# wooginawunan/multi-modal-uncertainty

Measured on AMD Instinct MI355X. Metric: image+text samples/sec/node, MMBT Food-101 bs=256 seq=512; ECE/NLL parity, higher is better.
Workload: dtype bf16

## Files before the change

multi-modal-uncertainty_amd/csrc/attention.hip:

```cpp
#include "mmu_common.h"
#include "mmu_internal.h"
#include <cstdlib>
#include <type_traits>
#include <utility>

namespace mmu {

constexpr float LOG2E = 1.4426950408889634f;
constexpr float LN2 = 0.6931471805599453f;
constexpr float NEG_INF = -__builtin_huge_valf();

static __device__ __forceinline__ uint32_t lowbias32(uint32_t x) {
  x ^= x >> 16; x *= 0x7feb352du; x ^= x >> 15; x *= 0x846ca68bu; x ^= x >> 16;
  return x;
}
static __device__ __forceinline__ uint32_t seed_for(uint64_t seed, int bh) {
  return lowbias32((uint32_t)seed ^ lowbias32((uint32_t)(seed >> 32) + 0x9E3779B9u * (uint32_t)(bh + 1)));
}
static __device__ __forceinline__ uint32_t drop_pair(uint32_t sbh, uint32_t q, uint32_t key, uint32_t Lp) {
  return lowbias32(((q * Lp + key) >> 1) ^ sbh);
}

static __device__ __forceinline__ float max3f(float a, float b, float c) {
  return __builtin_fmaxf(__builtin_fmaxf(a, b), c);
}
static __device__ __forceinline__ uint32_t bfi(uint32_t m, uint32_t a, uint32_t b) {
  return (m & a) | (~m & b);
}
static __device__ __forceinline__ uint32_t keepmask(uint32_t w, uint32_t pos) {
  uint32_t r;
  asm("v_bfe_i32 %0, %1, %2, 1" : "=v"(r) : "v"(w), "v"(pos));
  return r;
}
template <typename F, int... R>
static __device__ __forceinline__ void static_for(F&& f, std::integer_sequence<int, R...>) {
  (f(std::integral_constant<int, R>{}), ...);
}
template <int POS>
static __device__ __forceinline__ uint32_t keepmask(uint32_t w) {
  uint32_t r;
  asm("v_bfe_i32 %0, %1, %2, 1" : "=v"(r) : "v"(w), "n"(POS));
  return r;
}
static __host__ __device__ __forceinline__ uint32_t drop_thr(float p) { return (uint32_t)(p * 65536.0f + 0.5f); }

static __device__ __forceinline__ int fsw(int r) { return (((r >> 1) & 1) << 2) | ((r >> 3) & 3); }
static __device__ __forceinline__ int tile_off(int row, int chunk) { return row * 128 + ((chunk ^ fsw(row)) << 4); }

static __device__ __forceinline__ bf16x8 row_frag(const char* s, int row0, int ks, int l) {
  return *(const bf16x8*)(s + tile_off(row0 + (l & 31), 2 * ks + (l >> 5)));
}
static __device__ __forceinline__ bf16x8 tr_frag(const char* s, int row0, int col0, int l) {
  const int g = l >> 4, i = l & 15, q = i >> 2, p = i & 3, h = g >> 1;
  const int col = col0 + 16 * (g & 1) + 4 * p;
  const int r0 = row0 + 4 * h + q, r1 = r0 + 8;
  const int cb = col * 2;
  const char* a0 = s + tile_off(r0, cb >> 4) + (cb & 15);
  const char* a1 = s + tile_off(r1, cb >> 4) + (cb & 15);
  bf16x4 lo = __builtin_amdgcn_ds_read_tr16_b64_v4bf16((MMU_LDS(bf16x4)*)a0);
  bf16x4 hi = __builtin_amdgcn_ds_read_tr16_b64_v4bf16((MMU_LDS(bf16x4)*)a1);
  return __builtin_shufflevector(lo, hi, 0, 1, 2, 3, 4, 5, 6, 7);
}
static __device__ __forceinline__ bf16x8 acc_frag(const f32x16& a, int s) {
  bf16x8 r;
#pragma unroll
  for (int j = 0; j < 8; ++j) r[j] = f2bf(a[8 * s + j]);
  return r;
}
static __device__ __forceinline__ bf16x8 scale_frag(uint4 u, float sc) {
  bf16x8 v = *(bf16x8*)&u;
#pragma unroll
  for (int j = 0; j < 8; ++j) v[j] = f2bf(bf2f(v[j]) * sc);
  return v;
}

static __device__ __forceinline__ __amdgpu_buffer_rsrc_t urs(const void* base, int bytes) {
  const uint64_t a = (uint64_t)base;
  const uint32_t lo = __builtin_amdgcn_readfirstlane((uint32_t)a);
  const uint32_t hi = __builtin_amdgcn_readfirstlane((uint32_t)(a >> 32));
  const int n = __builtin_amdgcn_readfirstlane(bytes);
  return __builtin_amdgcn_make_buffer_rsrc((void*)(((uint64_t)hi << 32) | lo), 0, n, 0x00020000);
}

static __device__ __forceinline__ void dma16(__amdgpu_buffer_rsrc_t r, char* lds, uint32_t off) {
  __builtin_amdgcn_raw_ptr_buffer_load_lds(r, (MMU_LDS(void)*)lds, 16, off, 0, 0, 0);
}
static __device__ __forceinline__ __amdgpu_buffer_rsrc_t urs_at(const void* base, int bytes, int off) {
  return urs((const char*)base + off, bytes > off ? bytes - off : 0);
}
static __device__ __forceinline__ void dma4(__amdgpu_buffer_rsrc_t r, char* lds, uint32_t off) {
  __builtin_amdgcn_raw_ptr_buffer_load_lds(r, (MMU_LDS(void)*)lds, 4, off, 0, 0, 0);
}
static __device__ __forceinline__ void raw_barrier() {
  __builtin_amdgcn_s_barrier();
  asm volatile("" ::: "memory");
}

static __device__ __forceinline__ void block_coords(int& bx, int& bh) {
  const int gx = gridDim.x;
  const int wid = xcd_remap(blockIdx.y * gx + blockIdx.x, gx * gridDim.y);
  bh = wid / gx;
  bx = wid - bh * gx;
}

constexpr int FWD_NS = 2;
constexpr int FWD_TILE = 64 * 128;
constexpr int FWD_STAGE = 2 * FWD_TILE + 256;
constexpr int FWD_MAX_NKV = 9;

constexpr float DEFER_LOG2 = 8.0f;
constexpr uint32_t kDropMul24[8] = {0x9E3779u, 0x85EBCBu, 0xC2B2AFu, 0xA7D4EBu,
                                    0x965667u, 0xD3A265u, 0xFD7047u, 0xB55A4Fu};

static __device__ __forceinline__ uint32_t pair_draw(uint32_t hb, int i) {
  const uint32_t src = i ? __builtin_amdgcn_alignbit(hb, hb, 4 * i) : hb;
  const uint32_t x = __umul24(src, kDropMul24[i]);
  return x ^ (x >> 16);
}

static __device__ __forceinline__ int kperm(int i) {
  return (((i >> 2) & 1) << 4) | (((i >> 3) & 3) << 2) | (i & 3);
}

static __device__ __forceinline__ void drop_pair_zero(uint32_t hsh, uint32_t thr, uint32_t thr_hi, float e0,
                                                      float e1, float& o0, float& o1) {
  asm("v_cmp_le_u32 vcc, %[th], %[h]\n\t"
      "v_cndmask_b32 %[o1], 0, %[e1], vcc\n\t"
      "v_cmp_le_u16 vcc, %[t], %[h]\n\t"
      "v_cndmask_b32 %[o0], 0, %[e0], vcc"
      : [o0] "=&v"(o0), [o1] "=&v"(o1)
      : [e0] "v"(e0), [e1] "v"(e1), [h] "v"(hsh), [t] "s"(thr), [th] "s"(thr_hi)
      : "vcc");
}

static __device__ __forceinline__ void drop_pair_apply(uint32_t hsh, uint32_t thr, uint32_t thr_hi, float e0,
                                                       float e1, float& o0, float& o1, uint32_t& w) {
  asm("v_cmp_le_u32 vcc, %[th], %[h]\n\t"
      "v_cndmask_b32 %[o1], 0, %[e1], vcc\n\t"
      "v_addc_co_u32 %[w], vcc, %[w], %[w], vcc\n\t"
      "v_cmp_le_u16 vcc, %[t], %[h]\n\t"
      "v_cndmask_b32 %[o0], 0, %[e0], vcc\n\t"
      "v_addc_co_u32 %[w], vcc, %[w], %[w], vcc"
      : [o0] "=&v"(o0), [o1] "=&v"(o1), [w] "+v"(w)
      : [e0] "v"(e0), [e1] "v"(e1), [h] "v"(hsh), [t] "s"(thr), [th] "s"(thr_hi)
      : "vcc");
}

template <bool DROP, int WPE, bool NOHOIST, bool STORE = true>
__global__ __launch_bounds__(256) __attribute__((amdgpu_waves_per_eu(WPE))) void attn_fwd_v2_kernel(AttnParams p) {
  __shared__ __attribute__((aligned(16))) char smem[FWD_NS * FWD_STAGE + 4 * 32 * FWD_MAX_NKV * 8];
  uint64_t* kbuf_all = (uint64_t*)(smem + FWD_NS * FWD_STAGE);
  const int t = threadIdx.x, l = t & 63, l_ = l, h = l >> 5;
  const int w = __builtin_amdgcn_readfirstlane(t >> 6);
  int bx, bh;
  block_coords(bx, bh);
  const int b = bh / p.heads, hd = bh - b * p.heads;
  const int L = p.L, HD = p.heads * 64;
  const int q0w = bx * 128 + 32 * w, q = q0w + (l & 31);
  const bool wave_live = q0w < L;
  const bf16* base = p.qkv + (int64_t)b * L * p.ld_qkv + hd * 64;
  const uint32_t thr = drop_thr(p.drop_p), thr_hi = thr << 16;
  const int nkv = (L + 63) / 64;
  uint64_t* kbuf = kbuf_all + w * 32 * nkv;
  const bool store_bits = STORE && DROP && p.dropmask != nullptr;
  const uint32_t ctr = seed_for(mmu_eff_seed(p.seed, p.seed_off), bh) + 4u * (uint32_t)q * (uint32_t)nkv + 2u * (uint32_t)h;

  const void* kv_base = p.qkv + (int64_t)b * L * p.ld_qkv;
  const int kv_bytes = (int)(L * p.ld_qkv * 2);
  const void* m_base = p.keymask + (int64_t)b * L;
  bf16x8 qf[4];
#pragma unroll
  for (int ks = 0; ks < 4; ++ks) {
    uint4 u = q < L ? *(const uint4*)(base + (int64_t)q * p.ld_qkv + 16 * ks + 8 * h) : make_uint4(0, 0, 0, 0);
    qf[ks] = scale_frag(u, 0.125f);
// ... 106 lines not shown
      }
#pragma unroll
      for (int u = 0; u < 2; ++u) {
        if (PARTIAL && u == 1 && 64 * j + 32 * s2 + 8 >= L) break;
        const bf16x8 pf = acc_frag(sc[s2], u);
#pragma unroll
        for (int dt = 0; dt < 2; ++dt)
          o[dt] = __builtin_amdgcn_mfma_f32_32x32x16_bf16(tr_frag(Vs, 32 * s2 + 16 * u, 32 * dt, l), pf, o[dt], 0, 0, 0);
      }
    }
    if (store_bits) {
      const uint64_t mine = ((uint64_t)(wb[1] & 0xFFFFu) << (32 + 16 * h)) | ((uint64_t)(wb[0] & 0xFFFFu) << (16 * h));
      const uint32_t lo = (uint32_t)mine | (uint32_t)__shfl_xor((int)(uint32_t)mine, 32, 64);
      const uint32_t hi = (uint32_t)(mine >> 32) | (uint32_t)__shfl_xor((int)(uint32_t)(mine >> 32), 32, 64);
      if (h == 0) kbuf[(l & 31) * nkv + j] = ((uint64_t)hi << 32) | lo;
    }
  };

  asm volatile("s_waitcnt vmcnt(0)" ::: "memory");
  for (int j = 0; j < FWD_NS - 1 && j < nkv; ++j) issue(j);
  const int nfull = L / 64;
  auto step = [&](int j) {
    const int ahead = nkv - 1 - j < FWD_NS - 2 ? nkv - 1 - j : FWD_NS - 2;
    wait_for(ahead);
    raw_barrier();
    if (j + FWD_NS - 1 < nkv) issue(j + FWD_NS - 1);
  };
  static_assert(FWD_NS == 2, "the forward loop is unrolled by its ring depth");
  for (int j = 0; j < nfull; j += 2) {
    step(j);
    if (wave_live) tile(j, std::integral_constant<bool, false>{}, smem);
    if (j + 1 < nfull) {
      step(j + 1);
      if (wave_live) tile(j + 1, std::integral_constant<bool, false>{}, smem + FWD_STAGE);
    }
  }
  if (nfull < nkv) {
    step(nfull);
    if (wave_live) tile(nfull, std::integral_constant<bool, true>{}, smem + (nfull % FWD_NS) * FWD_STAGE);
  }
  raw_barrier();
  if (!wave_live) return;
  if (store_bits) {
    uint64_t* dst = p.dropmask + ((int64_t)bh * L + q0w) * nkv;
    const int rows = L - q0w < 32 ? L - q0w : 32;
    for (int i = l; i < rows * nkv; i += 64) dst[i] = kbuf[i];
  }
  const float l_run = (lsum[0] + lsum[1]) + (lsum[2] + lsum[3]);
  const float lsum_row = l_run + __shfl_xor(l_run, 32, 64);
  const float inv = (DROP ? 1.0f / (1.0f - p.drop_p) : 1.0f) / lsum_row;
  char* os = smem + w * 4096;
  const int qr = l & 31;
#pragma unroll
  for (int dt = 0; dt < 2; ++dt)
#pragma unroll
    for (int g = 0; g < 4; ++g) {
      const bf16x4 v = {f2bf(o[dt][4 * g] * inv), f2bf(o[dt][4 * g + 1] * inv), f2bf(o[dt][4 * g + 2] * inv),
                        f2bf(o[dt][4 * g + 3] * inv)};
      *(bf16x4*)(os + qr * 128 + (((4 * dt + g) ^ (qr & 7)) << 4) + 8 * h) = v;
    }
  if (h == 0 && q < L) p.lse[(int64_t)bh * L + q] = m_run + logf(lsum_row);
  asm volatile("s_waitcnt lgkmcnt(0)" ::: "memory");
  bf16* ob = p.out + hd * 64;
#pragma unroll
  for (int i = 0; i < 4; ++i) {
    const int r = (l >> 3) + 8 * i, c = l & 7;
    if (q0w + r < L)
      *(uint4*)(ob + ((int64_t)b * L + q0w + r) * p.ld_out + 8 * c) = *(const uint4*)(os + r * 128 + ((c ^ (r & 7)) << 4));
  }
}

void attention_fwd_launch(const AttnParams& p, hipStream_t s) {
  dim3 grid((p.L + 127) / 128, p.batch * p.heads);
  if (drop_thr(p.drop_p) && !p.dropmask) {
    hipLaunchKernelGGL((attn_fwd_v2_kernel<true, 3, true, false>), grid, dim3(256), 0, s, p);
  } else if (drop_thr(p.drop_p)) {
    hipLaunchKernelGGL((attn_fwd_v2_kernel<true, 2, false>), grid, dim3(256), 0, s, p);
  } else {
    hipLaunchKernelGGL((attn_fwd_v2_kernel<false, 3, false>), grid, dim3(256), 0, s, p);
  }
}

constexpr int DK_NS = 4;
constexpr int DK_TILE = 32 * 128;
constexpr int DK_ROWS = 32 * 4 + 32 * 4 + 32 * 8;
constexpr int DK_STAGE = 2 * DK_TILE + DK_ROWS;


template <bool DROP>
__global__ __launch_bounds__(128) __attribute__((amdgpu_waves_per_eu(2))) void attn_dkdv_dma_kernel(AttnParams p) {
  __shared__ __attribute__((aligned(16))) char smem[DK_NS * DK_STAGE];
  const int t = threadIdx.x, l = t & 63, h = l >> 5;
  const int w = __builtin_amdgcn_readfirstlane(t >> 6);
  int bx, bh;
  block_coords(bx, bh);
  const int b = bh / p.heads, hd = bh - b * p.heads;
  const int L = p.L, HD = p.heads * 64;
  const int k0w = bx * 64 + 32 * w, key = k0w + (l & 31);
  const bool wave_live = k0w < L, kv = key < L;
  const bool drop = DROP;
  const float zs = drop ? 1.0f / (1.0f - p.drop_p) : 1.0f;
  const int lane31 = l & 31;
  const int nkv = (L + 63) / 64;
  const float mkey = kv ? p.keymask[(int64_t)b * L + key] * LOG2E : NEG_INF;
  const bf16* base = p.qkv + (int64_t)b * L * p.ld_qkv + hd * 64;

  const void* q_base = p.qkv + (int64_t)b * L * p.ld_qkv;
  const int q_bytes = (int)(L * p.ld_qkv * 2);
  const void* do_base = p.dout + (int64_t)b * L * p.ld_do;
  const int do_bytes = (int)(L * p.ld_do * 2);
  const void* l_base = p.lse + (int64_t)bh * L;
  const void* d_base = p.delta + (int64_t)bh * L;
  const void* k_base = drop ? (const void*)(p.dropmask + (int64_t)bh * L * nkv) : nullptr;

  bf16x8 kf[4], vf[4];
#pragma unroll
  for (int ks = 0; ks < 4; ++ks) {
    uint4 u = kv ? *(const uint4*)(base + (int64_t)key * p.ld_qkv + HD + 16 * ks + 8 * h) : make_uint4(0, 0, 0, 0);
    uint4 v = kv ? *(const uint4*)(base + (int64_t)key * p.ld_qkv + 2 * HD + 16 * ks + 8 * h) : make_uint4(0, 0, 0, 0);
    kf[ks] = scale_frag(u, -0.125f);
    vf[ks] = *(bf16x8*)&v;
  }
  f32x16 dk[2], dv[2];
#pragma unroll
  for (int i = 0; i < 16; ++i) { dk[0][i] = 0.f; dk[1][i] = 0.f; dv[0][i] = 0.f; dv[1][i] = 0.f; }

  const int nq = (L + 31) / 32;
  uint32_t pc_off[4];
  const int ldr = w == 0 ? p.ld_qkv : p.ld_do;
#pragma unroll
  for (int pc = 0; pc < 4; ++pc) {
    const int row = 8 * pc + (l >> 3), c = (l & 7) ^ fsw(row);
    pc_off[pc] = (uint32_t)((row * ldr + hd * 64 + 8 * c) * 2);
  }
  const uint32_t row_off = (uint32_t)(16 * l), kw_off = (uint32_t)((((l >> 1) * nkv + bx) * 8) + 4 * (l & 1));
  auto issue = [&](int i) {
    char* st = smem + (i % DK_NS) * DK_STAGE;
    const int q0 = i * 32;
    if (w == 0) {
      const __amdgpu_buffer_rsrc_t rt = urs_at(q_base, q_bytes, q0 * p.ld_qkv * 2);
#pragma unroll
      for (int pc = 0; pc < 4; ++pc) dma16(rt, st + pc * 1024, pc_off[pc]);
      if (l < 8) {
        dma16(urs_at(l_base, L * 4, q0 * 4), st + 2 * DK_TILE, row_off);
        dma16(urs_at(d_base, L * 4, q0 * 4), st + 2 * DK_TILE + 128, row_off);
      }
    } else {
      const __amdgpu_buffer_rsrc_t rt = urs_at(do_base, do_bytes, q0 * p.ld_do * 2);
#pragma unroll
      for (int pc = 0; pc < 4; ++pc) dma16(rt, st + DK_TILE + pc * 1024, pc_off[pc]);
      dma4(urs_at(k_base, drop ? L * nkv * 8 : 0, q0 * nkv * 8), st + 2 * DK_TILE + 256, kw_off);
    }
  };
  auto wait_for = [&](int ahead) {
    if (w == 0) {
      if (ahead >= 2) asm volatile("s_waitcnt vmcnt(12)" ::: "memory");
      else if (ahead == 1) asm volatile("s_waitcnt vmcnt(6)" ::: "memory");
      else asm volatile("s_waitcnt vmcnt(0)" ::: "memory");
    } else {
      if (ahead >= 2) asm volatile("s_waitcnt vmcnt(10)" ::: "memory");
      else if (ahead == 1) asm volatile("s_waitcnt vmcnt(5)" ::: "memory");
      else asm volatile("s_waitcnt vmcnt(0)" ::: "memory");
    }
  };
  asm volatile("s_waitcnt vmcnt(0)" ::: "memory");
  for (int i = 0; i < DK_NS - 1 && i < nq; ++i) issue(i);
  auto qtile = [&](int i, auto sg_tag) {
    constexpr int SG = decltype(sg_tag)::value;
    const int ahead = nq - 1 - i < DK_NS - 2 ? nq - 1 - i : DK_NS - 2;
    wait_for(ahead);
    raw_barrier();
    if (i + DK_NS - 1 < nq) issue(i + DK_NS - 1);
    const char* st = smem + SG * DK_STAGE;
    const char* Qs = st;
    const char* Ds = st + DK_TILE;
    const float* lse = (const float*)(st + 2 * DK_TILE);
    const float* dlt = lse + 32;
    const uint32_t* kbit = (const uint32_t*)(st + 2 * DK_TILE + 256) + w;
    if (wave_live) {
      f32x4 l4[4], nd4[4];
      uint32_t kwr[16];
#pragma unroll
      for (int j = 0; j < 4; ++j) {
        l4[j] = *(const f32x4*)(lse + 8 * j + 4 * h);
        nd4[j] = *(const f32x4*)(dlt + 8 * j + 4 * h);
        if (DROP)
#pragma unroll
          for (int i2 = 0; i2 < 4; ++i2) kwr[4 * j + i2] = kbit[2 * (8 * j + 4 * h + i2)];
      }
      f32x16 sc, dp;
#pragma unroll
      for (int r = 0; r < 16; ++r) {
        sc[r] = l4[r >> 2][r & 3];
        dp[r] = nd4[r >> 2][r & 3];
      }
#pragma unroll
      for (int ks = 0; ks < 4; ++ks) {
        sc = __builtin_amdgcn_mfma_f32_32x32x16_bf16(row_frag(Qs, 0, ks, l), kf[ks], sc, 0, 0, 0);
        dp = __builtin_amdgcn_mfma_f32_32x32x16_bf16(row_frag(Ds, 0, ks, l), vf[ks], dp, 0, 0, 0);
      }
      f32x16 pz;
#pragma unroll
      for (int r = 0; r < 16; ++r) {
        const float pr = __builtin_amdgcn_exp2f(fmaf(sc[r], -LOG2E, mkey));
        if (DROP) {
          const uint32_t m = keepmask(kwr[r], lane31);
          pz[r] = __uint_as_float(m & __float_as_uint(pr));
          sc[r] = pr * __uint_as_float(bfi(m, __float_as_uint(dp[r]), __float_as_uint(nd4[r >> 2][r & 3])));
        } else {
          pz[r] = pr;
          sc[r] = pr * dp[r];
        }
      }
#pragma unroll
      for (int s2 = 0; s2 < 2; ++s2) {
        if (s2 == 1 && 32 * i + 16 >= L) break;
        bf16x8 pf = acc_frag(pz, s2), sf = acc_frag(sc, s2);
#pragma unroll
        for (int dt = 0; dt < 2; ++dt) {
          dv[dt] = __builtin_amdgcn_mfma_f32_32x32x16_bf16(pf, tr_frag(Ds, 16 * s2, 32 * dt, l), dv[dt], 0, 0, 0);
          dk[dt] = __builtin_amdgcn_mfma_f32_32x32x16_bf16(sf, tr_frag(Qs, 16 * s2, 32 * dt, l), dk[dt], 0, 0, 0);
        }
      }
    }
  };
  for (int i0 = 0; i0 < nq; i0 += DK_NS) {
    qtile(i0, std::integral_constant<int, 0>{});
    if (i0 + 1 < nq) qtile(i0 + 1, std::integral_constant<int, 1>{});
    if (i0 + 2 < nq) qtile(i0 + 2, std::integral_constant<int, 2>{});
    if (i0 + 3 < nq) qtile(i0 + 3, std::integral_constant<int, 3>{});
  }
  static_assert(DK_NS == 4, "the dK/dV loop is unrolled by its ring depth");
  const float dks = 0.125f * zs;
  if (p.colsum) {
    float* red = (float*)smem;
    raw_barrier();
#pragma unroll
    for (int dt = 0; dt < 2; ++dt) {
      float sk = 0.f, sv = 0.f;
#pragma unroll
      for (int r = 0; r < 16; ++r) {
        const bool ok = k0w + (r & 3) + 8 * (r >> 2) + 4 * h < L;
        sk += ok ? dk[dt][r] : 0.f;
        sv += ok ? dv[dt][r] : 0.f;
      }
      sk += __shfl_xor(sk, 32, 64);
      sv += __shfl_xor(sv, 32, 64);
      if (h == 0) {
        red[w * 128 + 32 * dt + l] = sk * dks;
        red[w * 128 + 64 + 32 * dt + l] = sv * zs;
      }
    }
    raw_barrier();
    if (t < 128) {
      const int nqb = (L + 127) / 128, nkb = (L + 63) / 64, B = p.batch;
      const float v = red[t] + red[128 + t];
      const int64_t row = (int64_t)nqb * B + (t < 64 ? 0 : (int64_t)nkb * B) + (int64_t)bx * B + b;
      p.colsum[row * HD + hd * 64 + (t & 63)] = v;
    }
  }
  if (!wave_live) return;
  bf16* outb = p.out + (int64_t)b * L * p.ld_out + hd * 64;
#pragma unroll
  for (int dt = 0; dt < 2; ++dt)
#pragma unroll
    for (int r = 0; r < 16; ++r) {
      const int kk = k0w + (r & 3) + 8 * (r >> 2) + 4 * h;
      if (kk < L) {
        const int64_t off = (int64_t)kk * p.ld_out + 32 * dt + (l & 31);
        outb[off + HD] = f2bf(dk[dt][r] * dks);
        outb[off + 2 * HD] = f2bf(dv[dt][r] * zs);
      }
    }
}

constexpr int DQ_NS = 3;
constexpr int DQ_TILE = 64 * 128;
constexpr int DQ_STAGE = 2 * DQ_TILE + 256 + 4 * 256;

__global__ __launch_bounds__(256) __attribute__((amdgpu_waves_per_eu(3))) void attn_dq_dma_kernel(AttnParams p) {
  __shared__ __attribute__((aligned(16))) char smem[DQ_NS * DQ_STAGE];
  const int t = threadIdx.x, l = t & 63, h = l >> 5;
  const int w = __builtin_amdgcn_readfirstlane(t >> 6);
  int bx, bh;
  block_coords(bx, bh);
  const int b = bh / p.heads, hd = bh - b * p.heads;
  const int L = p.L, HD = p.heads * 64;
  const int q0w = bx * 128 + 32 * w, q = q0w + (l & 31);
  const bool wave_live = q0w < L, qv = q < L;
  const bool drop = drop_thr(p.drop_p) != 0;
  const float zs = drop ? 1.0f / (1.0f - p.drop_p) : 1.0f;
  const int nkv = (L + 63) / 64;
  const bf16* base = p.qkv + (int64_t)b * L * p.ld_qkv + hd * 64;

  const void* kv_base = p.qkv + (int64_t)b * L * p.ld_qkv;
  const int kv_bytes = (int)(L * p.ld_qkv * 2);
  const void* m_base = p.keymask + (int64_t)b * L;
  const void* k_base = drop ? (const void*)(p.dropmask + (int64_t)bh * L * nkv) : nullptr;
  const int k_bytes = drop ? (int)(L * nkv * 8) : 0;

  bf16x8 qf[4], df[4];
  const bf16* dob = p.dout + ((int64_t)b * L + q) * p.ld_do + hd * 64;
#pragma unroll
  for (int ks = 0; ks < 4; ++ks) {
    uint4 u = qv ? *(const uint4*)(base + (int64_t)q * p.ld_qkv + 16 * ks + 8 * h) : make_uint4(0, 0, 0, 0);
    qf[ks] = scale_frag(u, 0.125f);
    uint4 v = qv ? *(const uint4*)(dob + 16 * ks + 8 * h) : make_uint4(0, 0, 0, 0);
    df[ks] = *(bf16x8*)&v;
  }
  float dsum = 0.f;
  {
    const bf16* ob = p.o + ((int64_t)b * L + q) * p.ld_o + hd * 64;
#pragma unroll
    for (int ks = 0; ks < 4; ++ks) {
      uint4 u = qv ? *(const uint4*)(ob + 16 * ks + 8 * h) : make_uint4(0, 0, 0, 0);
      const bf16x8 ov = *(bf16x8*)&u;
#pragma unroll
      for (int e = 0; e < 8; ++e) dsum = fmaf(bf2f(ov[e]), bf2f(df[ks][e]), dsum);
    }
    dsum += __shfl_xor(dsum, 32, 64);
    if (qv && h == 0) p.delta[(int64_t)bh * L + q] = -dsum / zs;
  }
  const float nlse2 = qv ? -p.lse[(int64_t)bh * L + q] * LOG2E : -__builtin_huge_valf();
  const float ndz = -dsum / zs;
  const uint32_t ndz_bits = __float_as_uint(ndz);
  f32x16 dq[2];
#pragma unroll
  for (int i = 0; i < 16; ++i) { dq[0][i] = 0.f; dq[1][i] = 0.f; }

  uint32_t kv_off[4];
#pragma unroll
  for (int pc = 0; pc < 4; ++pc) {
    const int piece = 4 * (w & 1) + pc;
    const int row = 8 * piece + (l >> 3), c = (l & 7) ^ fsw(row);
    kv_off[pc] = (uint32_t)((row * p.ld_qkv + (w < 2 ? HD : 2 * HD) + hd * 64 + 8 * c) * 2);
  }
  const uint32_t m_off = (uint32_t)(16 * l), kw_off = (uint32_t)(((q0w + (l >> 1)) * nkv * 8) + 4 * (l & 1));
  auto issue = [&](int j) {
    char* st = smem + (j % DQ_NS) * DQ_STAGE;
    const int k0 = j * 64;
    char* dst = st + (w < 2 ? 0 : DQ_TILE);
    const __amdgpu_buffer_rsrc_t rt = urs_at(kv_base, kv_bytes, k0 * p.ld_qkv * 2);
#pragma unroll
    for (int pc = 0; pc < 4; ++pc) dma16(rt, dst + (4 * (w & 1) + pc) * 1024, kv_off[pc]);
    if (w == 0 && l < 16) dma16(urs_at(m_base, L * 4, k0 * 4), st + 2 * DQ_TILE, m_off);
    dma4(urs_at(k_base, k_bytes, j * 8), st + 2 * DQ_TILE + 256 + w * 256, kw_off);
  };
  auto wait_for = [&](int ahead) {
    if (w == 0) {
      if (ahead >= 1) asm volatile("s_waitcnt vmcnt(6)" ::: "memory");
      else asm volatile("s_waitcnt vmcnt(0)" ::: "memory");
    } else {
      if (ahead >= 1) asm volatile("s_waitcnt vmcnt(5)" ::: "memory");
      else asm volatile("s_waitcnt vmcnt(0)" ::: "memory");
    }
  };
  asm volatile("s_waitcnt vmcnt(0)" ::: "memory");
  for (int j = 0; j < DQ_NS - 1 && j < nkv; ++j) issue(j);
  auto tile_step = [&](int j, auto sg_tag) {
    constexpr int SG = decltype(sg_tag)::value;
    const int ahead = nkv - 1 - j < DQ_NS - 2 ? nkv - 1 - j : DQ_NS - 2;
    wait_for(ahead);
    raw_barrier();
    if (j + DQ_NS - 1 < nkv) issue(j + DQ_NS - 1);
    const char* st = smem + SG * DQ_STAGE;
    const char* Ks = st;
    const char* Vs = st + DQ_TILE;
    const float* mk = (const float*)(st + 2 * DQ_TILE);
    const uint32_t* kwords = (const uint32_t*)(st + 2 * DQ_TILE + 256 + w * 256);
    if (wave_live) {
      const uint64_t kw = drop ? ((uint64_t)kwords[2 * (l & 31) + 1] << 32 | kwords[2 * (l & 31)]) : ~0ull;
      const uint64_t kwh = kw >> (4 * h);
#pragma unroll
      for (int st2 = 0; st2 < 2; ++st2) {
        if (st2 == 1 && 64 * j + 32 >= L) break;
        const uint32_t kw32 = (uint32_t)(kwh >> (32 * st2));
        f32x16 sc, dp;
#pragma unroll
        for (int g = 0; g < 4; ++g) {
          const f32x4 mv = *(const f32x4*)(mk + 32 * st2 + 8 * g + 4 * h);
#pragma unroll
          for (int e = 0; e < 4; ++e) {
            sc[4 * g + e] = mv[e];
            dp[4 * g + e] = ndz;
          }
        }
#pragma unroll
        for (int ks = 0; ks < 4; ++ks) {
          sc = __builtin_amdgcn_mfma_f32_32x32x16_bf16(row_frag(Ks, 32 * st2, ks, l), qf[ks], sc, 0, 0, 0);
          dp = __builtin_amdgcn_mfma_f32_32x32x16_bf16(row_frag(Vs, 32 * st2, ks, l), df[ks], dp, 0, 0, 0);
        }
        auto one = [&](auto r_tag) {
          constexpr int r = decltype(r_tag)::value;
          const float pr = __builtin_amdgcn_exp2f(fmaf(sc[r], LOG2E, nlse2));
          const uint32_t m = keepmask<(r & 3) + 8 * (r >> 2)>(kw32);
          sc[r] = pr * __uint_as_float(bfi(m, __float_as_uint(dp[r]), ndz_bits));
        };
        static_for(one, std::make_integer_sequence<int, 16>{});
#pragma unroll
        for (int s2 = 0; s2 < 2; ++s2) {
          bf16x8 sf = acc_frag(sc, s2);
#pragma unroll
          for (int dt = 0; dt < 2; ++dt)
            dq[dt] = __builtin_amdgcn_mfma_f32_32x32x16_bf16(tr_frag(Ks, 32 * st2 + 16 * s2, 32 * dt, l), sf, dq[dt],
                                                             0, 0, 0);
        }
      }
    }
    };
  for (int j0 = 0; j0 < nkv; j0 += DQ_NS) {
    tile_step(j0, std::integral_constant<int, 0>{});
    if (j0 + 1 < nkv) tile_step(j0 + 1, std::integral_constant<int, 1>{});
    if (j0 + 2 < nkv) tile_step(j0 + 2, std::integral_constant<int, 2>{});
  }
  if (p.colsum) {
    constexpr int RS = 68;
    static_assert(4 * 32 * RS * 4 <= DQ_NS * DQ_STAGE, "dQ column-sum rows exceed the ring's LDS");
    float* rows = (float*)smem;
    raw_barrier();
    float* mine = rows + w * 32 * RS + (l & 31) * RS;
    const float sc = qv ? 0.125f * zs : 0.f;
#pragma unroll
    for (int dt = 0; dt < 2; ++dt)
#pragma unroll
      for (int g = 0; g < 4; ++g)
        *(float4*)(mine + 32 * dt + 8 * g + 4 * h) =
            make_float4(dq[dt][4 * g] * sc, dq[dt][4 * g + 1] * sc, dq[dt][4 * g + 2] * sc, dq[dt][4 * g + 3] * sc);
    raw_barrier();
    if (t < 64) {
      float v = 0.f;
      for (int r = 0; r < 128; ++r) v += rows[r * RS + t];
      p.colsum[((int64_t)bx * p.batch + b) * HD + hd * 64 + t] = v;
    }
  }
  if (!qv) return;
  bf16* ob = p.out + ((int64_t)b * L + q) * p.ld_out + hd * 64;
#pragma unroll
  for (int dt = 0; dt < 2; ++dt)
#pragma unroll
    for (int g = 0; g < 4; ++g) {
      const float s = 0.125f * zs;
      bf16x4 v = {f2bf(dq[dt][4 * g] * s), f2bf(dq[dt][4 * g + 1] * s), f2bf(dq[dt][4 * g + 2] * s),
                  f2bf(dq[dt][4 * g + 3] * s)};
      *(bf16x4*)(ob + 32 * dt + 8 * g + 4 * h) = v;
    }
}

void attention_bwd_launch(const AttnParams& p, hipStream_t s) {
  hipLaunchKernelGGL(attn_dq_dma_kernel, dim3((p.L + 127) / 128, p.batch * p.heads), dim3(256), 0, s, p);
  if (drop_thr(p.drop_p))
    hipLaunchKernelGGL(attn_dkdv_dma_kernel<true>, dim3((p.L + 63) / 64, p.batch * p.heads), dim3(128), 0, s, p);
  else
    hipLaunchKernelGGL(attn_dkdv_dma_kernel<false>, dim3((p.L + 63) / 64, p.batch * p.heads), dim3(128), 0, s, p);
}

}
```

multi-modal-uncertainty_amd/csrc/capi.hip:

```cpp
#include <stdarg.h>
#include <stdio.h>
#include <map>
#include <tuple>
#include <mutex>
#include <string>
#include <vector>
#include "mmu_internal.h"
#include <cstdlib>
#include <cmath>

using namespace mmu;

static thread_local std::string g_err;

namespace mmu {
const uint64_t* g_seed_off = nullptr;
}

int mmu_set_seed_offset(const uint64_t* dev_counter) {
  g_seed_off = dev_counter;
  return 0;
}

static int fail(const char* fmt, ...) {
// ... 262 lines not shown
    splitk_epilogue_launch(pe, c_dtype == MMU_F32, tail_ws, m_main, tail_rows, tail_split, s);
  }
  if (cs_part) colsum_reduce_launch(cs_part, cs_parts, N, p.colsum, 1, s);
  if (p.splitk > 1) splitk_reduce_launch(p, (int)batch, s);
  if (timed) {
    (void)hipEventRecord(ev.second, s);
    std::lock_guard<std::mutex> lk(g_t.mu);
    g_t.used.push_back(ev);
    g_t.flops.push_back(2.0 * (double)M * (double)N * (double)K * (double)batch);
  }
  return check_launch("mmu_gemm");
}

int mmu_transpose_bf16_batched(const int64_t* jobs, int n_jobs, int64_t max_rows, int64_t max_cols,
                               mmu_stream_t stream) {
  if (!jobs || n_jobs <= 0 || n_jobs > 65535 || max_rows <= 0 || max_cols <= 0)
    return fail("mmu_transpose_bf16_batched: bad args");
  transpose_bf16_batched_launch(jobs, n_jobs, max_rows, max_cols, (hipStream_t)stream);
  return check_launch("mmu_transpose_bf16_batched");
}

int mmu_colsum_reduce(const float* partial, int64_t parts, int64_t N, float* out, int accumulate,
                      mmu_stream_t stream) {
  if (!partial || !out || parts <= 0 || N <= 0) return fail("mmu_colsum_reduce: bad args");
  colsum_reduce_launch(partial, parts, N, out, accumulate, (hipStream_t)stream);
  return check_launch("mmu_colsum_reduce");
}

int mmu_colsum_reduce_multi(int n, const float* const* partial, const int64_t* parts, float* const* out, int64_t N,
                            int accumulate, mmu_stream_t stream) {
  if (n <= 0 || n > COLSUM_MULTI || !partial || !parts || !out || N <= 0)
    return fail("mmu_colsum_reduce_multi: bad args (1 <= n <= %d)", COLSUM_MULTI);
  ColsumJobs jobs{};
  for (int z = 0; z < n; ++z) {
    if (!partial[z] || !out[z] || parts[z] <= 0) return fail("mmu_colsum_reduce_multi: bad job %d", z);
    jobs.part[z] = partial[z];
    jobs.parts[z] = parts[z];
    jobs.out[z] = out[z];
  }
  colsum_reduce_multi_launch(jobs, n, N, accumulate, (hipStream_t)stream);
  return check_launch("mmu_colsum_reduce_multi");
}

int mmu_colsum_bf16(const void* X, int64_t M, int64_t N, int64_t ldx, float* partial, float* out, int accumulate,
                    mmu_stream_t stream) {
  if (!X || !out || M <= 0 || N <= 0 || N % 8 || ldx % 8) return fail("mmu_colsum_bf16: bad args");
  colsum_bf16_launch((const bf16*)X, M, N, ldx, partial, out, accumulate, (hipStream_t)stream);
  return check_launch("mmu_colsum_bf16");
}

static int attn_common(int64_t ld_qkv, int64_t batch, int64_t L, int64_t heads, float drop_p) {
  if (batch <= 0 || L <= 0 || heads <= 0) return fail("attention: bad shape");
  if (ld_qkv < 3 * heads * 64 || ld_qkv % 8) return fail("attention: ld_qkv too small / unaligned");
  if (drop_p < 0.f || drop_p >= 1.f) return fail("attention: drop_p out of range");
  if ((int64_t)batch * heads > 65535 * 64) return fail("attention: batch*heads too large");
  if (L > 576) return fail("attention: L=%ld > 576 (the kernels stage ceil(L/64) <= 9 key tiles)", L);
  return 0;
}

int mmu_attention_fwd(const void* QKV, int64_t ld_qkv, const float* keymask, void* O, int64_t ld_o, float* LSE,
                      int64_t batch, int64_t L, int64_t heads, float drop_p, uint64_t seed, uint64_t* dropmask,
                      mmu_stream_t stream) {
  if (!QKV || !keymask || !O || !LSE) return fail("mmu_attention_fwd: null pointer");
  if (attn_common(ld_qkv, batch, L, heads, drop_p)) return 1;
  if (ld_o < heads * 64 || ld_o % 8) return fail("mmu_attention_fwd: bad ld_o");
  if (batch * heads > 65535) return fail("mmu_attention_fwd: batch*heads > 65535");
  AttnParams p{};
  p.qkv = (const bf16*)QKV; p.ld_qkv = ld_qkv; p.keymask = keymask; p.out = (bf16*)O; p.ld_out = ld_o;
  p.lse = LSE; p.batch = (int)batch; p.L = (int)L; p.heads = (int)heads; p.drop_p = drop_p; p.seed = seed;
  p.seed_off = g_seed_off;
  p.dropmask = dropmask;
  attention_fwd_launch(p, (hipStream_t)stream);
  return check_launch("mmu_attention_fwd");
}

int mmu_attention_bwd(const void* QKV, int64_t ld_qkv, const float* keymask, const void* O, int64_t ld_o,
                      const void* dO, int64_t ld_do, const float* LSE, float* delta, void* dQKV, int64_t ld_dqkv,
                      int64_t batch, int64_t L, int64_t heads, float drop_p, uint64_t seed,
                      const uint64_t* dropmask, float* dbias_parts, mmu_stream_t stream) {
  if (!QKV || !keymask || !O || !dO || !LSE || !delta || !dQKV) return fail("mmu_attention_bwd: null pointer");
  if ((uint32_t)(drop_p * 65536.0f + 0.5f) != 0 && !dropmask)
    return fail("mmu_attention_bwd: dropout needs the forward's dropmask");
  if (attn_common(ld_qkv, batch, L, heads, drop_p)) return 1;
  if (ld_dqkv < 3 * heads * 64 || ld_do % 8 || ld_o % 8 || ld_dqkv % 4) return fail("mmu_attention_bwd: bad ld");
  if (batch * heads > 65535) return fail("mmu_attention_bwd: batch*heads > 65535");
  AttnParams p{};
  p.qkv = (const bf16*)QKV; p.ld_qkv = ld_qkv; p.keymask = keymask; p.o = (const bf16*)O; p.ld_o = ld_o;
  p.dout = (const bf16*)dO; p.ld_do = ld_do; p.lse = (float*)LSE; p.delta = delta; p.out = (bf16*)dQKV;
  p.ld_out = ld_dqkv; p.batch = (int)batch; p.L = (int)L; p.heads = (int)heads; p.drop_p = drop_p; p.seed = seed;
  p.seed_off = g_seed_off;
  p.dropmask = (uint64_t*)dropmask;
  p.colsum = dbias_parts;
  attention_bwd_launch(p, (hipStream_t)stream);
  return check_launch("mmu_attention_bwd");
}

int mmu_layernorm_fwd(const void* X, const float* w, const float* b, void* Y, float* mean, float* rstd, int64_t rows,
                      int64_t H, float eps, int64_t group_rows, int64_t param_stride, mmu_stream_t stream) {
  if (!X || !w || !b || !Y) return fail("mmu_layernorm_fwd: null pointer");
  if ((mean == nullptr) != (rstd == nullptr)) return fail("mmu_layernorm_fwd: mean/rstd must both be given or NULL");
  if (rows <= 0 || H <= 0 || H % 256 || H > 1024) return fail("mmu_layernorm_fwd: H=%ld must be 256/512/768/1024", H);
  if (group_rows <= 0) group_rows = rows;
  if (param_stride < 0) return fail("mmu_layernorm_fwd: bad param_stride");
  layernorm_fwd_launch((const bf16*)X, w, b, (bf16*)Y, mean, rstd, rows, H, eps, group_rows, param_stride,
                       (hipStream_t)stream);
  return check_launch("mmu_layernorm_fwd");
}

int mmu_layernorm_bwd(const void* dY, const void* X, const float* mean, const float* rstd, const float* w, void* dX,
                      void* dXdrop, float drop_p, uint64_t seed, float* part_dw, float* part_db, float* part_dbias,
                      int64_t rows, int64_t H, int64_t rows_per_part, mmu_stream_t stream) {
  if (!dY || !X || !mean || !rstd || !w || !dX) return fail("mmu_layernorm_bwd: null pointer");
  if (rows <= 0 || H <= 0 || H % 256 || H > 1024 || rows_per_part <= 0) return fail("mmu_layernorm_bwd: bad shape");
  if (drop_p < 0.f || drop_p >= 1.f) return fail("mmu_layernorm_bwd: drop_p out of range");
  layernorm_bwd_launch((const bf16*)dY, X, false, mean, rstd, w, (bf16*)dX, (bf16*)dXdrop, nullptr, drop_p, seed,
                       g_seed_off, part_dw, part_db, part_dbias, rows, H, rows_per_part, (hipStream_t)stream);
  return check_launch("mmu_layernorm_bwd");
}

int mmu_layernorm_fwd_f32(const float* X, const float* w, const float* b, void* Y, float* Y32, float* mean,
                          float* rstd, int64_t rows, int64_t H, float eps, int64_t group_rows, int64_t param_stride,
                          mmu_stream_t stream) {
  if (!X || !w || !b || !Y) return fail("mmu_layernorm_fwd_f32: null pointer");
  if ((mean == nullptr) != (rstd == nullptr)) return fail("mmu_layernorm_fwd_f32: mean/rstd must both be given or NULL");
  if (rows <= 0 || H <= 0 || H % 256 || H > 1024) return fail("mmu_layernorm_fwd_f32: H=%ld must be 256/512/768/1024", H);
  if (group_rows <= 0) group_rows = rows;
  if (param_stride < 0) return fail("mmu_layernorm_fwd_f32: bad param_stride");
  layernorm_fwd32_launch(X, w, b, (bf16*)Y, Y32, mean, rstd, rows, H, eps, group_rows, param_stride,
                         (hipStream_t)stream);
  return check_launch("mmu_layernorm_fwd_f32");
}

int mmu_layernorm_bwd_f32(const void* dY, const float* X, const float* mean, const float* rstd, const float* w,
                          void* dX, void* dXdrop, float drop_p, uint64_t seed, float* part_dw, float* part_db,
                          float* part_dbias, int64_t rows, int64_t H, int64_t rows_per_part, mmu_stream_t stream) {
  if (!dY || !X || !mean || !rstd || !w || !dX) return fail("mmu_layernorm_bwd_f32: null pointer");
  if (rows <= 0 || H <= 0 || H % 256 || H > 1024 || rows_per_part <= 0) return fail("mmu_layernorm_bwd_f32: bad shape");
  if (drop_p < 0.f || drop_p >= 1.f) return fail("mmu_layernorm_bwd_f32: drop_p out of range");
  layernorm_bwd_launch((const bf16*)dY, X, true, mean, rstd, w, (bf16*)dX, (bf16*)dXdrop, nullptr, drop_p, seed,
                       g_seed_off, part_dw, part_db, part_dbias, rows, H, rows_per_part, (hipStream_t)stream);
  return check_launch("mmu_layernorm_bwd_f32");
}

int mmu_layernorm_bwd_res(const void* dY, const void* X, const float* mean, const float* rstd, const float* w,
                          const void* dRes, void* dX, float* part_dw, float* part_db, float* part_dbias, int64_t rows,
                          int64_t H, int64_t rows_per_part, mmu_stream_t stream) {
  if (!dY || !X || !mean || !rstd || !w || !dX || !dRes) return fail("mmu_layernorm_bwd_res: null pointer");
  if (rows <= 0 || H <= 0 || H % 256 || H > 1024 || rows_per_part <= 0) return fail("mmu_layernorm_bwd_res: bad shape");
  layernorm_bwd_launch((const bf16*)dY, X, false, mean, rstd, w, (bf16*)dX, nullptr, (const bf16*)dRes, 0.f, 0,
                       nullptr, part_dw, part_db, part_dbias, rows, H, rows_per_part, (hipStream_t)stream);
  return check_launch("mmu_layernorm_bwd_res");
}

static int seqattn_check(const char* what, int64_t ld_qkv, int64_t S, int64_t N, int64_t heads, int64_t D) {
  if (S <= 0 || N <= 0 || heads <= 0) return fail("%s: bad shape", what);
  if (D != 64 && D != 128 && D != 256) return fail("%s: head_dim %ld not in {64, 128, 256}", what, D);
  if (ld_qkv < 3 * heads * D || ld_qkv % 8) return fail("%s: ld_qkv too small / unaligned", what);
  if (N * heads > 65535) return fail("%s: N*heads > 65535", what);
  return 0;
}

int mmu_seqattn_fwd(const void* QKV, int64_t ld_qkv, void* O, int64_t ld_o, float* LSE2, int64_t S, int64_t N,
                    int64_t heads, int64_t head_dim, mmu_stream_t stream) {
  if (!QKV || !O || !LSE2) return fail("mmu_seqattn_fwd: null pointer");
  if (seqattn_check("mmu_seqattn_fwd", ld_qkv, S, N, heads, head_dim)) return 1;
  if (ld_o < heads * head_dim || ld_o % 4) return fail("mmu_seqattn_fwd: bad ld_o");
  SeqAttnParams p{};
// ... 477 lines not shown
```

Baseline: 1652.

## Widen dK/dV attention backward to four waves with LDS-staged vectorized output

The dK/dV backward kernel goes from 2 waves (64 keys) to 4 waves (128 keys) per block. The Q/dO tile DMA is split across wave pairs, so each staged Q/dO tile serves twice as many keys and fewer blocks reload the same rows. The scattered scalar dK/dV stores are replaced by staging in LDS and transposed ds_read_tr16 reads, giving 16-byte global stores, which requires ld_dqkv to be a multiple of 8. Buffer-load-to-LDS is moved to inline asm with raw descriptors, and the dropout-mask and delta loads are software-pipelined per row group. The waves_per_eu hint is raised, which risks register pressure.

Result: no change. 1660 (median of 6 runs) (+0.5%).

```diff
diff --git a/multi-modal-uncertainty_amd/csrc/attention.hip b/multi-modal-uncertainty_amd/csrc/attention.hip
--- a/multi-modal-uncertainty_amd/csrc/attention.hip
+++ b/multi-modal-uncertainty_amd/csrc/attention.hip
@@ -90,6 +90,29 @@
 }
 static __device__ __forceinline__ void dma4(__amdgpu_buffer_rsrc_t r, char* lds, uint32_t off) {
   __builtin_amdgcn_raw_ptr_buffer_load_lds(r, (MMU_LDS(void)*)lds, 4, off, 0, 0, 0);
+}
+typedef uint32_t u32x4 __attribute__((ext_vector_type(4)));
+static __device__ __forceinline__ u32x4 urs4_at(const void* base, int bytes, int off) {
+  const uint64_t a = (uint64_t)((const char*)base + off);
+  u32x4 d;
+  d[0] = __builtin_amdgcn_readfirstlane((uint32_t)a);
+  d[1] = __builtin_amdgcn_readfirstlane((uint32_t)(a >> 32)) & 0xFFFFu;
+  d[2] = __builtin_amdgcn_readfirstlane(bytes > off ? bytes - off : 0);
+  d[3] = 0x00020000u;
+  return d;
+}
+static __device__ __forceinline__ uint32_t lds_addr(const void* a) {
+  return (uint32_t)(uintptr_t)(MMU_LDS(const char)*)(const char*)a;
+}
+static __device__ __forceinline__ void dma16a(u32x4 r, const char* lds, uint32_t off) {
+  asm volatile("s_mov_b32 m0, %2\n\ts_nop 0\n\tbuffer_load_dwordx4 %0, %1, 0 offen lds"
+               :: "v"(off), "s"(r), "s"(__builtin_amdgcn_readfirstlane(lds_addr(lds)))
+               : "memory");
+}
+static __device__ __forceinline__ void dma4a(u32x4 r, const char* lds, uint32_t off) {
+  asm volatile("s_mov_b32 m0, %2\n\ts_nop 0\n\tbuffer_load_dword %0, %1, 0 offen lds"
+               :: "v"(off), "s"(r), "s"(__builtin_amdgcn_readfirstlane(lds_addr(lds)))
+               : "memory");
 }
 static __device__ __forceinline__ void raw_barrier() {
   __builtin_amdgcn_s_barrier();
@@ -362,13 +385,16 @@
 }
 
 constexpr int DK_NS = 4;
+constexpr int DK_WAVES = 4;
 constexpr int DK_TILE = 32 * 128;
-constexpr int DK_ROWS = 32 * 4 + 32 * 4 + 32 * 8;
+constexpr int DK_ROWS = 32 * 4 + 32 * 4 + 2 * 32 * 8;
 constexpr int DK_STAGE = 2 * DK_TILE + DK_ROWS;
-
+constexpr int DK_OUT = 2 * 64 * 64;
+static_assert(DK_WAVES * DK_OUT + DK_WAVES * 128 * 4 <= DK_NS * DK_STAGE,
+              "dK/dV output staging and column-sum rows exceed the ring's LDS");
 
 template <bool DROP>
-__global__ __launch_bounds__(128) __attribute__((amdgpu_waves_per_eu(2))) void attn_dkdv_dma_kernel(AttnParams p) {
+__global__ __launch_bounds__(64 * DK_WAVES) __attribute__((amdgpu_waves_per_eu(3))) void attn_dkdv_dma_kernel(AttnParams p) {
   __shared__ __attribute__((aligned(16))) char smem[DK_NS * DK_STAGE];
   const int t = threadIdx.x, l = t & 63, h = l >> 5;
   const int w = __builtin_amdgcn_readfirstlane(t >> 6);
@@ -376,7 +402,7 @@
   block_coords(bx, bh);
   const int b = bh / p.heads, hd = bh - b * p.heads;
   const int L = p.L, HD = p.heads * 64;
-  const int k0w = bx * 64 + 32 * w, key = k0w + (l & 31);
+  const int k0w = bx * (32 * DK_WAVES) + 32 * w, key = k0w + (l & 31);
   const bool wave_live = k0w < L, kv = key < L;
   const bool drop = DROP;
   const float zs = drop ? 1.0f / (1.0f - p.drop_p) : 1.0f;
@@ -406,42 +432,33 @@
   for (int i = 0; i < 16; ++i) { dk[0][i] = 0.f; dk[1][i] = 0.f; dv[0][i] = 0.f; dv[1][i] = 0.f; }
 
   const int nq = (L + 31) / 32;
-  uint32_t pc_off[4];
-  const int ldr = w == 0 ? p.ld_qkv : p.ld_do;
-#pragma unroll
-  for (int pc = 0; pc < 4; ++pc) {
-    const int row = 8 * pc + (l >> 3), c = (l & 7) ^ fsw(row);
+  uint32_t pc_off[2];
+  const int ldr = w < 2 ? p.ld_qkv : p.ld_do;
+#pragma unroll
+  for (int pc = 0; pc < 2; ++pc) {
+    const int row = 8 * (2 * (w & 1) + pc) + (l >> 3), c = (l & 7) ^ fsw(row);
     pc_off[pc] = (uint32_t)((row * ldr + hd * 64 + 8 * c) * 2);
   }
-  const uint32_t row_off = (uint32_t)(16 * l), kw_off = (uint32_t)((((l >> 1) * nkv + bx) * 8) + 4 * (l & 1));
+  const uint32_t sm_off = w < 2 ? (uint32_t)(16 * l) : (uint32_t)((((l >> 1) * nkv + 2 * bx + (w - 2)) * 8) + 4 * (l & 1));
   auto issue = [&](int i) {
     char* st = smem + (i % DK_NS) * DK_STAGE;
     const int q0 = i * 32;
-    if (w == 0) {
-      const __amdgpu_buffer_rsrc_t rt = urs_at(q_base, q_bytes, q0 * p.ld_qkv * 2);
-#pragma unroll
-      for (int pc = 0; pc < 4; ++pc) dma16(rt, st + pc * 1024, pc_off[pc]);
-      if (l < 8) {
-        dma16(urs_at(l_base, L * 4, q0 * 4), st + 2 * DK_TILE, row_off);
-        dma16(urs_at(d_base, L * 4, q0 * 4), st + 2 * DK_TILE + 128, row_off);
-      }
+    if (w < 2) {
+      const u32x4 rt = urs4_at(q_base, q_bytes, q0 * p.ld_qkv * 2);
+#pragma unroll
+      for (int pc = 0; pc < 2; ++pc) dma16a(rt, st + (2 * w + pc) * 1024, pc_off[pc]);
+      if (l < 8) dma16a(urs4_at(w == 0 ? l_base : d_base, L * 4, q0 * 4), st + 2 * DK_TILE + w * 128, sm_off);
     } else {
-      const __amdgpu_buffer_rsrc_t rt = urs_at(do_base, do_bytes, q0 * p.ld_do * 2);
-#pragma unroll
-      for (int pc = 0; pc < 4; ++pc) dma16(rt, st + DK_TILE + pc * 1024, pc_off[pc]);
-      dma4(urs_at(k_base, drop ? L * nkv * 8 : 0, q0 * nkv * 8), st + 2 * DK_TILE + 256, kw_off);
+      const u32x4 rt = urs4_at(do_base, do_bytes, q0 * p.ld_do * 2);
+#pragma unroll
+      for (int pc = 0; pc < 2; ++pc) dma16a(rt, st + DK_TILE + (2 * (w - 2) + pc) * 1024, pc_off[pc]);
+      dma4a(urs4_at(k_base, drop ? L * nkv * 8 : 0, q0 * nkv * 8), st + 2 * DK_TILE + 256 + (w - 2) * 256, sm_off);
     }
   };
   auto wait_for = [&](int ahead) {
-    if (w == 0) {
-      if (ahead >= 2) asm volatile("s_waitcnt vmcnt(12)" ::: "memory");
-      else if (ahead == 1) asm volatile("s_waitcnt vmcnt(6)" ::: "memory");
-      else asm volatile("s_waitcnt vmcnt(0)" ::: "memory");
-    } else {
-      if (ahead >= 2) asm volatile("s_waitcnt vmcnt(10)" ::: "memory");
-      else if (ahead == 1) asm volatile("s_waitcnt vmcnt(5)" ::: "memory");
-      else asm volatile("s_waitcnt vmcnt(0)" ::: "memory");
-    }
+    if (ahead >= 2) asm volatile("s_waitcnt vmcnt(6)" ::: "memory");
+    else if (ahead == 1) asm volatile("s_waitcnt vmcnt(3)" ::: "memory");
+    else asm volatile("s_waitcnt vmcnt(0)" ::: "memory");
   };
   asm volatile("s_waitcnt vmcnt(0)" ::: "memory");
   for (int i = 0; i < DK_NS - 1 && i < nq; ++i) issue(i);
@@ -456,17 +473,13 @@
     const char* Ds = st + DK_TILE;
     const float* lse = (const float*)(st + 2 * DK_TILE);
     const float* dlt = lse + 32;
-    const uint32_t* kbit = (const uint32_t*)(st + 2 * DK_TILE + 256) + w;
+    const uint32_t* kbit = (const uint32_t*)(st + 2 * DK_TILE + 256 + (w >> 1) * 256) + (w & 1);
     if (wave_live) {
       f32x4 l4[4], nd4[4];
-      uint32_t kwr[16];
 #pragma unroll
       for (int j = 0; j < 4; ++j) {
         l4[j] = *(const f32x4*)(lse + 8 * j + 4 * h);
         nd4[j] = *(const f32x4*)(dlt + 8 * j + 4 * h);
-        if (DROP)
-#pragma unroll
-          for (int i2 = 0; i2 < 4; ++i2) kwr[4 * j + i2] = kbit[2 * (8 * j + 4 * h + i2)];
       }
       f32x16 sc, dp;
 #pragma unroll
@@ -480,18 +493,35 @@
         dp = __builtin_amdgcn_mfma_f32_32x32x16_bf16(row_frag(Ds, 0, ks, l), vf[ks], dp, 0, 0, 0);
       }
       f32x16 pz;
-#pragma unroll
-      for (int r = 0; r < 16; ++r) {
-        const float pr = __builtin_amdgcn_exp2f(fmaf(sc[r], -LOG2E, mkey));
-        if (DROP) {
-          const uint32_t m = keepmask(kwr[r], lane31);
-          pz[r] = __uint_as_float(m & __float_as_uint(pr));
-          sc[r] = pr * __uint_as_float(bfi(m, __float_as_uint(dp[r]), __float_as_uint(nd4[r >> 2][r & 3])));
-        } else {
-          pz[r] = pr;
-          sc[r] = pr * dp[r];
+      int zo = 4 * h;
+      if (DROP) asm("" : "+v"(zo));
+      f32x4 ndg[2];
+      uint32_t kwg[2][4];
+      auto load_group = [&](auto j_tag) {
+        constexpr int j = decltype(j_tag)::value;
+        ndg[j & 1] = *(const f32x4*)(dlt + 8 * j + zo);
+#pragma unroll
+        for (int i2 = 0; i2 < 4; ++i2) kwg[j & 1][i2] = kbit[2 * (8 * j + i2 + zo)];
+      };
+      if (DROP) load_group(std::integral_constant<int, 0>{});
+      auto group = [&](auto j_tag) {
+        constexpr int j = decltype(j_tag)::value;
+        if (DROP && j < 3) load_group(std::integral_constant<int, (j + 1) & 3>{});
+#pragma unroll
+        for (int e = 0; e < 4; ++e) {
+          const int r = 4 * j + e;
+          const float pr = __builtin_amdgcn_exp2f(fmaf(sc[r], -LOG2E, mkey));
+          if (DROP) {
+            const uint32_t m = keepmask(kwg[j & 1][e], lane31);
+            pz[r] = __uint_as_float(m & __float_as_uint(pr));
+            sc[r] = pr * __uint_as_float(bfi(m, __float_as_uint(dp[r]), __float_as_uint(ndg[j & 1][e])));
+          } else {
+            pz[r] = pr;
+            sc[r] = pr * dp[r];
+          }
         }
-      }
+      };
+      static_for(group, std::make_integer_sequence<int, 4>{});
 #pragma unroll
       for (int s2 = 0; s2 < 2; ++s2) {
         if (s2 == 1 && 32 * i + 16 >= L) break;
@@ -512,9 +542,9 @@
   }
   static_assert(DK_NS == 4, "the dK/dV loop is unrolled by its ring depth");
   const float dks = 0.125f * zs;
+  raw_barrier();
   if (p.colsum) {
-    float* red = (float*)smem;
-    raw_barrier();
+    float* red = (float*)(smem + DK_WAVES * DK_OUT);
 #pragma unroll
     for (int dt = 0; dt < 2; ++dt) {
       float sk = 0.f, sv = 0.f;
@@ -532,26 +562,48 @@
       }
     }
     raw_barrier();
-    if (t < 128) {
-      const int nqb = (L + 127) / 128, nkb = (L + 63) / 64, B = p.batch;
-      const float v = red[t] + red[128 + t];
-      const int64_t row = (int64_t)nqb * B + (t < 64 ? 0 : (int64_t)nkb * B) + (int64_t)bx * B + b;
-      p.colsum[row * HD + hd * 64 + (t & 63)] = v;
+    const int j = t >> 7, tt = t & 127;
+    const int nqb = (L + 127) / 128, nkb = (L + 63) / 64, B = p.batch, kb = 2 * bx + j;
+    if (kb < nkb) {
+      const float v = red[2 * j * 128 + tt] + red[(2 * j + 1) * 128 + tt];
+      const int64_t row = (int64_t)nqb * B + (tt < 64 ? 0 : (int64_t)nkb * B) + (int64_t)kb * B + b;
+      p.colsum[row * HD + hd * 64 + (tt & 63)] = v;
     }
   }
   if (!wave_live) return;
+  char* os = smem + w * DK_OUT;
+#pragma unroll
+  for (int dt = 0; dt < 2; ++dt)
+#pragma unroll
+    for (int g = 0; g < 4; ++g) {
+      const int c = 32 * dt + lane31;
+      const int off = c * 64 + (((2 * g + h) ^ ((c >> 1) & 7)) << 3);
+      const bf16x4 a = {f2bf(dk[dt][4 * g] * dks), f2bf(dk[dt][4 * g + 1] * dks), f2bf(dk[dt][4 * g + 2] * dks),
+                        f2bf(dk[dt][4 * g + 3] * dks)};
+      const bf16x4 c4 = {f2bf(dv[dt][4 * g] * zs), f2bf(dv[dt][4 * g + 1] * zs), f2bf(dv[dt][4 * g + 2] * zs),
+                         f2bf(dv[dt][4 * g + 3] * zs)};
+      *(bf16x4*)(os + off) = a;
+      *(bf16x4*)(os + DK_OUT / 2 + off) = c4;
+    }
+  asm volatile("s_waitcnt lgkmcnt(0)" ::: "memory");
   bf16* outb = p.out + (int64_t)b * L * p.ld_out + hd * 64;
-#pragma unroll
-  for (int dt = 0; dt < 2; ++dt)
-#pragma unroll
-    for (int r = 0; r < 16; ++r) {
-      const int kk = k0w + (r & 3) + 8 * (r >> 2) + 4 * h;
-      if (kk < L) {
-        const int64_t off = (int64_t)kk * p.ld_out + 32 * dt + (l & 31);
-        outb[off + HD] = f2bf(dk[dt][r] * dks);
-        outb[off + 2 * HD] = f2bf(dv[dt][r] * zs);
-      }
-    }
+  const int i16 = l & 15, q4 = i16 >> 2, p4 = i16 & 3, gq = l >> 4;
+#pragma unroll
+  for (int s = 0; s < 4; ++s) {
+    const int kk = k0w + 16 * (s & 1) + i16;
+    const int cb = 32 * (s >> 1) + 8 * gq;
+    const int ch = 4 * (s & 1) + p4;
+    const int r0 = cb + q4, r1 = r0 + 4;
+    const int o0 = r0 * 64 + ((ch ^ ((r0 >> 1) & 7)) << 3), o1 = r1 * 64 + ((ch ^ ((r1 >> 1) & 7)) << 3);
+#pragma unroll
+    for (int m = 0; m < 2; ++m) {
+      const char* im = os + m * (DK_OUT / 2);
+      const bf16x4 lo = __builtin_amdgcn_ds_read_tr16_b64_v4bf16((MMU_LDS(bf16x4)*)(im + o0));
+      const bf16x4 hi = __builtin_amdgcn_ds_read_tr16_b64_v4bf16((MMU_LDS(bf16x4)*)(im + o1));
+      const bf16x8 v = __builtin_shufflevector(lo, hi, 0, 1, 2, 3, 4, 5, 6, 7);
+      if (kk < L) *(bf16x8*)(outb + (int64_t)kk * p.ld_out + (m + 1) * HD + cb) = v;
+    }
+  }
 }
 
 constexpr int DQ_NS = 3;
@@ -620,11 +672,11 @@
     char* st = smem + (j % DQ_NS) * DQ_STAGE;
     const int k0 = j * 64;
     char* dst = st + (w < 2 ? 0 : DQ_TILE);
-    const __amdgpu_buffer_rsrc_t rt = urs_at(kv_base, kv_bytes, k0 * p.ld_qkv * 2);
-#pragma unroll
-    for (int pc = 0; pc < 4; ++pc) dma16(rt, dst + (4 * (w & 1) + pc) * 1024, kv_off[pc]);
-    if (w == 0 && l < 16) dma16(urs_at(m_base, L * 4, k0 * 4), st + 2 * DQ_TILE, m_off);
-    dma4(urs_at(k_base, k_bytes, j * 8), st + 2 * DQ_TILE + 256 + w * 256, kw_off);
+    const u32x4 rt = urs4_at(kv_base, kv_bytes, k0 * p.ld_qkv * 2);
+#pragma unroll
+    for (int pc = 0; pc < 4; ++pc) dma16a(rt, dst + (4 * (w & 1) + pc) * 1024, kv_off[pc]);
+    if (w == 0 && l < 16) dma16a(urs4_at(m_base, L * 4, k0 * 4), st + 2 * DQ_TILE, m_off);
+    dma4a(urs4_at(k_base, k_bytes, j * 8), st + 2 * DQ_TILE + 256 + w * 256, kw_off);
   };
   auto wait_for = [&](int ahead) {
     if (w == 0) {
@@ -728,10 +780,11 @@
 
 void attention_bwd_launch(const AttnParams& p, hipStream_t s) {
   hipLaunchKernelGGL(attn_dq_dma_kernel, dim3((p.L + 127) / 128, p.batch * p.heads), dim3(256), 0, s, p);
+  const dim3 dkdv_grid((p.L + 32 * DK_WAVES - 1) / (32 * DK_WAVES), p.batch * p.heads);
   if (drop_thr(p.drop_p))
-    hipLaunchKernelGGL(attn_dkdv_dma_kernel<true>, dim3((p.L + 63) / 64, p.batch * p.heads), dim3(128), 0, s, p);
+    hipLaunchKernelGGL(attn_dkdv_dma_kernel<true>, dkdv_grid, dim3(64 * DK_WAVES), 0, s, p);
   else
-    hipLaunchKernelGGL(attn_dkdv_dma_kernel<false>, dim3((p.L + 63) / 64, p.batch * p.heads), dim3(128), 0, s, p);
-}
-
-}
+    hipLaunchKernelGGL(attn_dkdv_dma_kernel<false>, dkdv_grid, dim3(64 * DK_WAVES), 0, s, p);
+}
+
+}
diff --git a/multi-modal-uncertainty_amd/csrc/capi.hip b/multi-modal-uncertainty_amd/csrc/capi.hip
--- a/multi-modal-uncertainty_amd/csrc/capi.hip
+++ b/multi-modal-uncertainty_amd/csrc/capi.hip
@@ -368,7 +368,7 @@
   if ((uint32_t)(drop_p * 65536.0f + 0.5f) != 0 && !dropmask)
     return fail("mmu_attention_bwd: dropout needs the forward's dropmask");
   if (attn_common(ld_qkv, batch, L, heads, drop_p)) return 1;
-  if (ld_dqkv < 3 * heads * 64 || ld_do % 8 || ld_o % 8 || ld_dqkv % 4) return fail("mmu_attention_bwd: bad ld");
+  if (ld_dqkv < 3 * heads * 64 || ld_do % 8 || ld_o % 8 || ld_dqkv % 8) return fail("mmu_attention_bwd: bad ld");
   if (batch * heads > 65535) return fail("mmu_attention_bwd: batch*heads > 65535");
   AttnParams p{};
   p.qkv = (const bf16*)QKV; p.ld_qkv = ld_qkv; p.keymask = keymask; p.o = (const bf16*)O; p.ld_o = ld_o;
```
